# symek/facedeform

Hardware: AMD Instinct MI355X
Metric: deformed Mverts/sec at 256 ctrl pts, 1/2/4/8 MI355X vs host-CPU ref (higher is better)
Workload: dtype f32

## Files before the change

### facedeform_amd/csrc/fd_capi.hip

```cpp
#include <algorithm>
#include <atomic>
#include <cstdarg>
#include <cstdio>
#include <cstdlib>
#include <cstring>
#include <initializer_list>
#include <new>
#include <vector>

#include "fd_internal.h"

using namespace fd;

struct GraphKey {
    int M, kind, term, nparams;
    double params[4];
    const void *A, *rest, *rec32;
};

struct fd_batch;
struct fd_ctx {
    int device = 0;
    hipStream_t own_stream = nullptr;
    hipStream_t stream_ = nullptr;
    int eval_precision = FD_EVAL_FP32;
    int eval_variant = 0;
    int output = FD_OUTPUT_POSITION;
    int solver = FD_SOLVER_AUTO;
    int imported_layers = 0;
    uint64_t rig_build_id = 0;
    const float *rest_src = nullptr;
    bool prefer_lu = false;
    unsigned long long model_gen = 0;
    bool last_spd = false;
    bool last_small = false;
    bool last_nopivot = false;
    bool last_reg = false;

    int M = 0, kind = FD_KERNEL_GAUSSIAN_QNN, term = FD_TERM_LINEAR, nparams = 0;
    double params[4] = {1.0, 5.0, 0.0, 0.0};
    bool points_set = false;
    bool build_pending = false;
    bool built = false;
    bool have_report = false;
    fd_report report{};
    bool have_factor = false;
    bool factor_grouped = false;
    bool deltas_only = false;
    hipGraphExec_t resolve_exec = nullptr;

    int cap_M = 0;
// ... 8 lines not shown
    MfmaTile *d_tiles = nullptr;
    MfmaTileH *d_tiles16 = nullptr;
    double *d_ns = nullptr;
    DevModel *d_model = nullptr;
    DevModel *h_model = nullptr;
    BatchSlot *d_slot = nullptr;
    BatchSlot h_slot{};
    uint64_t alloc_gen = 0;
    hipEvent_t wait_event = nullptr;
    hipStream_t wait_stream = nullptr;
    struct fd_batch *wait_batch = nullptr;
    hipEvent_t tev0 = nullptr, tev_mid = nullptr, tev1 = nullptr;
    ModelHeader *h_header = nullptr;
    int *h_status = nullptr;
    int *d_status_alias = nullptr;
    hipEvent_t status_ev = nullptr;
    hipEvent_t status_poll = nullptr;
    bool status_inflight = false;
    int sticky_rc = FD_OK;

    int64_t cap_N = 0;
    float *d_P = nullptr, *d_dist2 = nullptr, *d_fall = nullptr;
    float *d_tu = nullptr, *d_tv = nullptr, *d_nrm = nullptr;
    int64_t cap_vec = 0, cap_vecP = 0;
    float *d_vec = nullptr, *d_vecP = nullptr;
    int64_t cap_iters = 0;
    int *d_iters = nullptr;
    size_t cap_adj = 0;
    double *d_adj = nullptr;
    int64_t mesh_N = 0, mesh_cap = 0;
    bool mesh_has_dist2 = false, mesh_has_frames = false;
    float *m_P = nullptr, *m_dist2 = nullptr, *m_tu = nullptr, *m_tv = nullptr, *m_nrm = nullptr;
    float *m_out = nullptr, *m_fall = nullptr;

    hipEvent_t ev0 = nullptr, ev_mid = nullptr, ev1 = nullptr;

    hipGraphExec_t build_exec = nullptr;
    bool use_graph = true;
    GraphKey graph_key{}, resolve_key{};
    char err[512] = {0};
};

struct ShotScratch {
    void *d = nullptr;
    size_t cap = 0;
    hipEvent_t consumed_ev = nullptr;
    bool consumed = false;
    hipEvent_t eval_ev = nullptr;
    bool eval_pending = false;
};

struct fd_batch {
    int n = 0;
    int device = 0;
    fd_ctx *ctxs[kMaxBatch] = {};
    uint64_t gens[kMaxBatch] = {};
    BatchSlot *d_slots = nullptr;
    PointSrc src{};
    bool have_src = false;
    hipEvent_t ev0 = nullptr, ev_mid = nullptr, ev1 = nullptr;
    hipGraphExec_t exec = nullptr;
    bool use_graph = true;
    GraphKey key{};
    hipStream_t waited_stream = nullptr;
    hipEvent_t status_ev = nullptr;
    struct SharedSet {
// ... 304 lines not shown
    }
    if (strncmp(prop.gcnArchName, "gfx950", 6) != 0) {
        set_err(nullptr, "fd_create: device %d is %s; kernels are built for gfx950 (MI355X) only",
                dev, prop.gcnArchName);
        delete ctx;
        return nullptr;
    }
    bool ok = true;
    ok = ok && hipEventCreate(&ctx->ev0) == hipSuccess && hipEventCreate(&ctx->ev_mid) == hipSuccess &&
         hipEventCreate(&ctx->ev1) == hipSuccess;
    ok = ok && hipMalloc((void **)&ctx->d_model, sizeof(DevModel)) == hipSuccess;
    ok = ok && hipMalloc((void **)&ctx->d_slot, sizeof(BatchSlot)) == hipSuccess;
    ok = ok && hipHostMalloc((void **)&ctx->h_model, sizeof(DevModel), hipHostMallocDefault) == hipSuccess;
    ok = ok && hipHostMalloc((void **)&ctx->h_header, sizeof(ModelHeader), hipHostMallocDefault) == hipSuccess;
    ok = ok && hipHostMalloc((void **)&ctx->h_status, sizeof(int), hipHostMallocDefault) == hipSuccess;
    if (ok && hipHostGetDevicePointer((void **)&ctx->d_status_alias, ctx->h_status, 0) != hipSuccess) { (void)hipGetLastError(); ctx->d_status_alias = nullptr; }
    ok = ok && hipEventCreateWithFlags(&ctx->status_ev, hipEventDisableTiming) == hipSuccess;
    if (ok) ok = hipMemset(ctx->d_model, 0, sizeof(DevModel)) == hipSuccess;
    if (!ok) {
        set_err(nullptr, "fd_create: device resource allocation failed: %s",
                hipGetErrorString(hipGetLastError()));
        fd_destroy(ctx);
        return nullptr;
    }
    ctx->tev0 = ctx->ev0; ctx->tev_mid = ctx->ev_mid; ctx->tev1 = ctx->ev1;
    return ctx;
}

void fd_destroy(fd_ctx *ctx)
{
    if (!ctx) return;
    (void)hipSetDevice(ctx->device);
    if (ctx->stream_ || ctx->own_stream) (void)hipStreamSynchronize(cur_stream(ctx));
    void *bufs[] = {ctx->d_rest, ctx->d_delta, ctx->d_centres, ctx->d_radii, ctx->d_W, ctx->d_A,
                    ctx->d_X, ctx->d_ipiv, ctx->d_moves, ctx->d_rec32, ctx->d_rec64, ctx->d_tiles, ctx->d_tiles16, ctx->d_ns, ctx->d_model, ctx->d_slot,
                    ctx->d_P, ctx->d_dist2, ctx->d_fall, ctx->d_tu, ctx->d_tv, ctx->d_nrm, ctx->d_vec, ctx->d_vecP, ctx->d_iters, ctx->d_adj,
                    ctx->m_P, ctx->m_dist2, ctx->m_tu, ctx->m_tv, ctx->m_nrm, ctx->m_out, ctx->m_fall};
    for (void *p : bufs) if (p) (void)hipFree(p);
    if (ctx->h_model) (void)hipHostFree(ctx->h_model);
    if (ctx->h_header) (void)hipHostFree(ctx->h_header);
    if (ctx->h_status) (void)hipHostFree(ctx->h_status);
    if (ctx->status_ev) (void)hipEventDestroy(ctx->status_ev);
    if (ctx->build_exec) (void)hipGraphExecDestroy(ctx->build_exec);
    if (ctx->resolve_exec) (void)hipGraphExecDestroy(ctx->resolve_exec);
    if (ctx->ev0) (void)hipEventDestroy(ctx->ev0);
    if (ctx->ev_mid) (void)hipEventDestroy(ctx->ev_mid);
    if (ctx->ev1) (void)hipEventDestroy(ctx->ev1);
    if (ctx->own_stream) (void)hipStreamDestroy(ctx->own_stream);
    delete ctx;
}

int fd_set_stream(fd_ctx *ctx, void *hip_stream)
{
    if (!ctx) return FD_E_INVALID;
    int rc = use_device(ctx);
    if (rc) return rc;
    if (ctx->stream_ || ctx->own_stream) FD_HIP(ctx, hipStreamSynchronize(cur_stream(ctx)));
    ctx->stream_ = (hipStream_t)hip_stream;
    return FD_OK;
}

int fd_synchronize(fd_ctx *ctx)
{
    if (!ctx) return FD_E_INVALID;
    int rc = use_device(ctx);
    if (rc) return rc;
// ... 834 lines not shown
    unsigned char *d_mask = nullptr;
    hipError_t e = hipMalloc((void **)&d_P, sizeof(float) * 3 * (size_t)N);
    if (e == hipSuccess) e = hipMalloc((void **)&d_off, sizeof(int64_t) * (size_t)(N + 1));
    if (e == hipSuccess) e = hipMalloc((void **)&d_nb, sizeof(int) * (size_t)(E > 0 ? E : 1));
    if (e == hipSuccess) e = hipMalloc((void **)&d_mask, (size_t)N);
    if (e == hipSuccess && M > 0) e = hipMalloc((void **)&d_rig, sizeof(float) * 3 * (size_t)M);
    if (e == hipSuccess) e = hipMemcpyAsync(d_P, P, sizeof(float) * 3 * (size_t)N, hipMemcpyHostToDevice, s);
    if (e == hipSuccess) e = hipMemcpyAsync(d_off, offsets, sizeof(int64_t) * (size_t)(N + 1), hipMemcpyHostToDevice, s);
    if (e == hipSuccess && E > 0) e = hipMemcpyAsync(d_nb, neighbours, sizeof(int) * (size_t)E, hipMemcpyHostToDevice, s);
    if (e == hipSuccess && M > 0) e = hipMemcpyAsync(d_rig, rig_xyz, sizeof(float) * 3 * (size_t)M, hipMemcpyHostToDevice, s);
    if (e == hipSuccess) e = launch_capture_islands(d_P, N, d_off, d_nb, d_rig, M, max_edges, d_mask, s);
    if (e == hipSuccess) e = hipMemcpyAsync(mask, d_mask, (size_t)N, hipMemcpyDeviceToHost, s);
    if (e == hipSuccess) e = hipStreamSynchronize(s);
    for (void *p : {(void *)d_P, (void *)d_off, (void *)d_nb, (void *)d_mask, (void *)d_rig}) if (p) (void)hipFree(p);
    if (e != hipSuccess) { set_err(ctx, "fd_capture_islands failed: %s", hipGetErrorString(e)); return FD_E_DEVICE; }
    return FD_OK;
}

void *fd_host_alloc(size_t bytes)
{
    void *p = nullptr;
    if (hipHostMalloc(&p, bytes ? bytes : 1, hipHostMallocDefault) != hipSuccess) {
        set_err(nullptr, "fd_host_alloc(%zu) failed: %s", bytes, hipGetErrorString(hipGetLastError()));
        return nullptr;
    }
    return p;
}

void fd_host_free(void *p)
{
    if (p) (void)hipHostFree(p);
}

int fd_mesh_set(fd_ctx *ctx, int64_t N, const float *P, const float *dist2, const float *tu, const float *tv,
                const float *nrm)
{
    if (!ctx) return FD_E_INVALID;
    if (N <= 0 || !P) { set_err(ctx, "fd_mesh_set: need N > 0 and P"); return FD_E_INVALID; }
    if (!frames_ok(tu, tv, nrm)) { set_err(ctx, "fd_mesh_set: tu, tv, nrm must be all set or all NULL"); return FD_E_INVALID; }
    int rc = use_device(ctx);
    if (rc) return rc;
    ctx->mesh_N = 0;
    if (N > ctx->mesh_cap) {
        if ((rc = dev_alloc(ctx, &ctx->m_P, (size_t)N * 3))) return rc;
        if (ctx->m_dist2) { (void)hipFree(ctx->m_dist2); ctx->m_dist2 = nullptr; }
        if (ctx->m_tu) { (void)hipFree(ctx->m_tu); ctx->m_tu = nullptr; }
        if (ctx->m_tv) { (void)hipFree(ctx->m_tv); ctx->m_tv = nullptr; }
        if (ctx->m_nrm) { (void)hipFree(ctx->m_nrm); ctx->m_nrm = nullptr; }
        if (ctx->m_out) { (void)hipFree(ctx->m_out); ctx->m_out = nullptr; }
        if (ctx->m_fall) { (void)hipFree(ctx->m_fall); ctx->m_fall = nullptr; }
        ctx->mesh_cap = N;
    }
    if (dist2 && !ctx->m_dist2 && (rc = dev_alloc(ctx, &ctx->m_dist2, (size_t)ctx->mesh_cap))) return rc;
    if (tu && !ctx->m_tu) {
        if ((rc = dev_alloc(ctx, &ctx->m_tu, (size_t)ctx->mesh_cap * 3))) return rc;
        if ((rc = dev_alloc(ctx, &ctx->m_tv, (size_t)ctx->mesh_cap * 3))) return rc;
        if ((rc = dev_alloc(ctx, &ctx->m_nrm, (size_t)ctx->mesh_cap * 3))) return rc;
    }
    hipStream_t s = cur_stream(ctx);
    const size_t b3 = sizeof(float) * 3 * (size_t)N, b1 = sizeof(float) * (size_t)N;
    FD_HIP(ctx, hipMemcpyAsync(ctx->m_P, P, b3, hipMemcpyHostToDevice, s));
    if (dist2) FD_HIP(ctx, hipMemcpyAsync(ctx->m_dist2, dist2, b1, hipMemcpyHostToDevice, s));
    if (tu) {
        FD_HIP(ctx, hipMemcpyAsync(ctx->m_tu, tu, b3, hipMemcpyHostToDevice, s));
        FD_HIP(ctx, hipMemcpyAsync(ctx->m_tv, tv, b3, hipMemcpyHostToDevice, s));
        FD_HIP(ctx, hipMemcpyAsync(ctx->m_nrm, nrm, b3, hipMemcpyHostToDevice, s));
    }
    FD_HIP(ctx, hipStreamSynchronize(s));
    ctx->mesh_N = N;
    ctx->mesh_has_dist2 = dist2 != nullptr;
    ctx->mesh_has_frames = tu != nullptr;
    return FD_OK;
}

int64_t fd_mesh_size(const fd_ctx *ctx) { return ctx ? ctx->mesh_N : 0; }

int fd_deform_mesh(fd_ctx *ctx, float *P_out, float *falloff_out, float radius2, float falloffrate)
{
    if (!ctx) return FD_E_INVALID;
    if (ctx->mesh_N <= 0) { set_err(ctx, "fd_deform_mesh: fd_mesh_set has not been called"); return FD_E_INVALID; }
    if (!P_out) { set_err(ctx, "fd_deform_mesh: P_out is NULL"); return FD_E_INVALID; }
    if (!ctx->built && !ctx->build_pending) { set_err(ctx, "fd_deform_mesh: no successfully built model"); return FD_E_NOT_BUILT; }
    int rc = use_device(ctx);
    if (rc) return rc;
    const int64_t N = ctx->mesh_N;
    hipStream_t s = cur_stream(ctx);
    const float *d2 = ctx->mesh_has_dist2 ? ctx->m_dist2 : nullptr;
    const float *tu = ctx->mesh_has_frames ? ctx->m_tu : nullptr, *tv = ctx->mesh_has_frames ? ctx->m_tv : nullptr,
                *nr = ctx->mesh_has_frames ? ctx->m_nrm : nullptr;
    if (host_is_pinned(P_out) && (!falloff_out || host_is_pinned(falloff_out))) {
        void *zo = nullptr, *zf = nullptr;
        bool ok = hipHostGetDevicePointer(&zo, P_out, 0) == hipSuccess;
        if (ok && falloff_out) ok = hipHostGetDevicePointer(&zf, falloff_out, 0) == hipSuccess;
        if (ok) {
            rc = fd_deform_dev_stream(ctx, s, N, ctx->m_P, (float *)zo, d2, (float *)zf, tu, tv, nr, radius2, falloffrate);
            if (rc) return rc;
            FD_HIP(ctx, hipStreamSynchronize(s));
            return FD_OK;
        }
        (void)hipGetLastError();
    }
    if (!ctx->m_out && (rc = dev_alloc(ctx, &ctx->m_out, (size_t)ctx->mesh_cap * 3))) return rc;
    if (falloff_out && !ctx->m_fall && (rc = dev_alloc(ctx, &ctx->m_fall, (size_t)ctx->mesh_cap))) return rc;
    const size_t b3 = sizeof(float) * 3 * (size_t)N, b1 = sizeof(float) * (size_t)N;
    if (falloff_out && (d2 || radius2 < 0.f)) FD_HIP(ctx, hipMemcpyAsync(ctx->m_fall, falloff_out, b1, hipMemcpyHostToDevice, s));
    rc = fd_deform_dev_stream(ctx, s, N, ctx->m_P, ctx->m_out, d2, falloff_out ? ctx->m_fall : nullptr, tu, tv, nr, radius2,
                              falloffrate);
    if (rc) return rc;
    FD_HIP(ctx, hipMemcpyAsync(P_out, ctx->m_out, b3, hipMemcpyDeviceToHost, s));
    if (falloff_out) FD_HIP(ctx, hipMemcpyAsync(falloff_out, ctx->m_fall, b1, hipMemcpyDeviceToHost, s));
    FD_HIP(ctx, hipStreamSynchronize(s));
    return FD_OK;
}

int fd_mesh_capture(fd_ctx *ctx, const int64_t *offsets, const int *neighbours, int M, const float *rig_xyz,
                    int max_edges, int T, const float *tri_xyz, float radius2, int dofalloff, float *dist2_out)
{
    if (!ctx) return FD_E_INVALID;
    const int64_t N = ctx->mesh_N;
    if (N <= 0) { set_err(ctx, "fd_mesh_capture: fd_mesh_set has not been called"); return FD_E_INVALID; }
    if (!offsets || M < 0 || T < 0 || max_edges < 0 || (M > 0 && !rig_xyz) || (T > 0 && !tri_xyz)) {
        set_err(ctx, "fd_mesh_capture: bad sizes or NULL arrays");
        return FD_E_INVALID;
    }
    const int64_t E = offsets[N];
    if (offsets[0] != 0 || E < 0 || (E > 0 && !neighbours)) { set_err(ctx, "fd_mesh_capture: bad adjacency"); return FD_E_INVALID; }
    int rc = use_device(ctx);
    if (rc) return rc;
    if (!ctx->m_dist2 && (rc = dev_alloc(ctx, &ctx->m_dist2, (size_t)ctx->mesh_cap))) return rc;
    hipStream_t s = cur_stream(ctx);
    float *d_rig = nullptr, *d_tri = nullptr;
    int64_t *d_off = nullptr;
    int *d_nb = nullptr;
    unsigned char *d_mask = nullptr;
    hipError_t e = hipMalloc((void **)&d_off, sizeof(int64_t) * (size_t)(N + 1));
    if (e == hipSuccess) e = hipMalloc((void **)&d_nb, sizeof(int) * (size_t)(E > 0 ? E : 1));
    if (e == hipSuccess) e = hipMalloc((void **)&d_mask, (size_t)N);
    if (e == hipSuccess) e = hipMalloc((void **)&d_rig, sizeof(float) * 3 * (size_t)(M > 0 ? M : 1));
    if (e == hipSuccess) e = hipMalloc((void **)&d_tri, sizeof(float) * 9 * (size_t)(T > 0 ? T : 1));
    if (e == hipSuccess) e = hipMemcpyAsync(d_off, offsets, sizeof(int64_t) * (size_t)(N + 1), hipMemcpyHostToDevice, s);
    if (e == hipSuccess && E > 0) e = hipMemcpyAsync(d_nb, neighbours, sizeof(int) * (size_t)E, hipMemcpyHostToDevice, s);
    if (e == hipSuccess && M > 0) e = hipMemcpyAsync(d_rig, rig_xyz, sizeof(float) * 3 * (size_t)M, hipMemcpyHostToDevice, s);
    if (e == hipSuccess && T > 0) e = hipMemcpyAsync(d_tri, tri_xyz, sizeof(float) * 9 * (size_t)T, hipMemcpyHostToDevice, s);
    if (e == hipSuccess) e = launch_capture_islands(ctx->m_P, N, d_off, d_nb, d_rig, M, max_edges, d_mask, s);
    if (e == hipSuccess) e = launch_capture_dist2(ctx->m_P, N, d_mask, d_tri, T, radius2, dofalloff, ctx->m_dist2, s);
    if (e == hipSuccess && dist2_out) e = hipMemcpyAsync(dist2_out, ctx->m_dist2, sizeof(float) * (size_t)N, hipMemcpyDeviceToHost, s);
    if (e == hipSuccess) e = hipStreamSynchronize(s);
    for (void *p : {(void *)d_off, (void *)d_nb, (void *)d_mask, (void *)d_rig, (void *)d_tri}) if (p) (void)hipFree(p);
    if (e != hipSuccess) { (void)hipGetLastError(); set_err(ctx, "fd_mesh_capture failed: %s", hipGetErrorString(e)); return FD_E_DEVICE; }
    ctx->mesh_has_dist2 = true;
    return FD_OK;
}

int fd_mesh_get_dist2(fd_ctx *ctx, float *dist2_out)
{
    if (!ctx || !dist2_out) return FD_E_INVALID;
    if (ctx->mesh_N <= 0 || !ctx->mesh_has_dist2 || !ctx->m_dist2) { set_err(ctx, "fd_mesh_get_dist2: the mesh has no dist2 array"); return FD_E_INVALID; }
    int rc = use_device(ctx);
    if (rc) return rc;
    hipStream_t s = cur_stream(ctx);
    FD_HIP(ctx, hipMemcpyAsync(dist2_out, ctx->m_dist2, sizeof(float) * (size_t)ctx->mesh_N, hipMemcpyDeviceToHost, s));
    FD_HIP(ctx, hipStreamSynchronize(s));
    return FD_OK;
}

static int require_built(fd_ctx *ctx, const char *who)
{
    if (ctx->build_pending) {
        int rc = fd_build_result(ctx, nullptr);
        if (rc) return rc;
    }
    if (!ctx->built) { set_err(ctx, "%s: no successfully built model", who); return FD_E_NOT_BUILT; }
    return FD_OK;
}

int fd_model_centres(const fd_ctx *ctx) { return ctx ? model_centres(ctx) : 0; }

int fd_get_weights(fd_ctx *ctx, double *W, double *radii)
{
    if (!ctx || !W) return FD_E_INVALID;
    int rc = use_device(ctx);
    if (rc) return rc;
    if ((rc = require_built(ctx, "fd_get_weights"))) return rc;
    const int n = model_centres(ctx);
    FD_HIP(ctx, hipMemcpyAsync(W, ctx->d_W, sizeof(double) * 3 * (size_t)(n + 4), hipMemcpyDeviceToHost, cur_stream(ctx)));
    if (radii) FD_HIP(ctx, hipMemcpyAsync(radii, ctx->d_radii, sizeof(double) * (size_t)n, hipMemcpyDeviceToHost, cur_stream(ctx)));
    FD_HIP(ctx, hipStreamSynchronize(cur_stream(ctx)));
    return FD_OK;
}

static size_t model_bytes_for(int M)
{
    return sizeof(ModelHeader) + sizeof(double) * ((size_t)M * 3 + (size_t)M + (size_t)(M + 4) * 3);
}

// ... 1209 lines not shown
}

int fd_batch_set_shared_factor(fd_batch *b, int on)
{
    if (!b) return FD_E_INVALID;
    b->shared_factor = on ? 1 : 0;
    return FD_OK;
}

int fd_batch_last_build_shared_factor(const fd_batch *b) { return b ? b->last_shared_factor : 0; }

const char *fd_shared_ml_build_kernel_name(int M, int layers, int frames) { return ml_shared_kernel_name(M, layers, frames); }

int fd_batch_set_shared_lu(fd_batch *b, int on)
{
    if (!b) return FD_E_INVALID;
    b->shared_lu = on ? 1 : 0;
    return FD_OK;
}

const char *fd_shared_qnn_build_kernel_name(int M, int frames) { return qnn_shared_kernel_name(M, frames); }

int fd_batch_size(const fd_batch *b) { return b ? b->n : 0; }

const char *fd_shared_kernel_name(int M, int frames, int kind)
{
    const bool takes = (kind == FD_KERNEL_THIN_PLATE || kind == FD_KERNEL_GAUSSIAN || kind == FD_KERNEL_GAUSSIAN_QNN) && M > 0 && round_up(M, kRecPad) >= 32 &&
                       frames >= 1 && frames <= kMaxBatch;
    return takes ? shared_kernel_name(round_up(M, kRecPad), frames, kind) : "";
}

}

#include "fd_shot_dev.h"

struct fd_shot_dev {
    fd_ctx *engine = nullptr;
    hipStream_t work = nullptr, copy = nullptr;
    float *d_rig = nullptr;
    size_t cap_rig = 0;
    int M = 0, F = 0;
    float *d_vecs = nullptr;
    int64_t cap_vecs = 0;
    const float *v_in[3] = {nullptr, nullptr, nullptr};
    struct Set {
        float *d = nullptr;
        size_t bytes = 0;
        hipEvent_t eval_ev = nullptr, delivered_ev = nullptr;
        bool delivering = false;
    } sets[2];
    int set_frames = 0;
    int64_t set_Np = 0;
    bool set_fall = false;
    int set_nvec = 0;
    char err[512] = {0};
};

static void shot_err(fd_shot_dev *sd, const char *fmt, ...)
{
    va_list ap;
    va_start(ap, fmt);
    vsnprintf(sd->err, sizeof(sd->err), fmt, ap);
    va_end(ap);
}

#define FD_SHIP(sd, call)                                                                          \
    do {                                                                                           \
        hipError_t e_ = (call);                                                                    \
// ... 135 lines not shown
        }
        (void)hipGetLastError();
        for (auto &st : sd->sets) { if (st.d) (void)hipFree(st.d); st.d = nullptr; }
    }
    shot_err(sd, "hipMalloc of the shot's staging sets failed: %s", hipGetErrorString(hipErrorOutOfMemory));
    return 0;
}

int fd_shot_dev_wait(fd_shot_dev *sd, int set)
{
    if (!sd || set < 0 || set > 1) return FD_E_INVALID;
    if (!sd->sets[set].delivering) return FD_OK;
    sd->sets[set].delivering = false;
    FD_SHIP(sd, hipEventSynchronize(sd->sets[set].delivered_ev));
    return FD_OK;
}

struct ShotMesh { int64_t N; const float *P, *d2, *tu, *tv, *nr; };
static ShotMesh shot_mesh(const fd_ctx *e)
{
    ShotMesh m{e->mesh_N, e->m_P, e->mesh_has_dist2 ? e->m_dist2 : nullptr, nullptr, nullptr, nullptr};
    if (e->mesh_has_frames) { m.tu = e->m_tu; m.tv = e->m_tv; m.nr = e->m_nrm; }
    return m;
}

int fd_shot_dev_eval(fd_shot_dev *sd, fd_batch *b, int set, int fp64, int multilayer, float radius2, float falloffrate)
{
    if (!sd || !b || set < 0 || set > 1) return FD_E_INVALID;
    const int n = b->n;
    if (!sd->sets[set].d || n > sd->set_frames) { shot_err(sd, "fd_shot_dev_eval: no staging set for %d frames", n); return FD_E_INVALID; }
    int rc = fd_shot_dev_wait(sd, set);
    if (rc) return rc;
    const ShotMesh m = shot_mesh(sd->engine);
    if (m.N <= 0 || shot_pad(m.N) != sd->set_Np) { shot_err(sd, "fd_shot_dev_eval: the staging sets were laid out for another mesh"); return FD_E_INVALID; }
    float *P_out[kMaxBatch], *fall[kMaxBatch], *vo[3][kMaxBatch];
    for (int i = 0; i < n; ++i) {
        P_out[i] = shot_slice_P(sd, set, i);
        fall[i] = shot_slice_fall(sd, set, i);
    }
    fd_batch_vectors vec{};
    vec.struct_size = (int)sizeof(vec);
    int which = 0;
    for (int k = 0; k < 3; ++k) {
        if (!sd->v_in[k]) continue;
        for (int i = 0; i < n; ++i) vo[k][i] = shot_slice_vec(sd, set, which, i);
        ++which;
    }
    if (sd->v_in[0]) { vec.N = sd->v_in[0]; vec.N_out = vo[0]; }
    if (sd->v_in[1]) { vec.tu = sd->v_in[1]; vec.tu_out = vo[1]; }
    if (sd->v_in[2]) { vec.tv = sd->v_in[2]; vec.tv_out = vo[2]; }
    const bool with_vec = which > 0;
    if (sd->set_fall && (m.d2 || radius2 < 0.f))
        FD_SHIP(sd, hipMemsetAsync(shot_slice_fall(sd, set, 0), 0, sizeof(float) * (size_t)n * (size_t)sd->set_Np, sd->work));
    float *const *fo = sd->set_fall ? fall : nullptr;
    if (with_vec) {
        auto call = fp64 ? (multilayer ? fd_batch_deform_vectors_shared_ml_fp64_dev : fd_batch_deform_vectors_shared_fp64_dev)
                         : (multilayer ? fd_batch_deform_vectors_shared_ml_dev : fd_batch_deform_vectors_shared_dev);
        rc = call(b, sd->work, m.N, m.P, P_out, m.d2, fo, m.tu, m.tv, m.nr, radius2, falloffrate, &vec);
    } else {
        auto call = fp64 ? (multilayer ? fd_batch_deform_shared_ml_fp64_dev : fd_batch_deform_shared_fp64_dev)
                         : (multilayer ? fd_batch_deform_shared_ml_dev : fd_batch_deform_shared_dev);
        rc = call(b, sd->work, m.N, m.P, P_out, m.d2, fo, m.tu, m.tv, m.nr, radius2, falloffrate);
    }
    if (rc) { shot_err(sd, "%s", b->err); return rc; }
    FD_SHIP(sd, hipEventRecord(sd->sets[set].eval_ev, sd->work));
    return FD_OK;
}

int fd_shot_dev_eval_fp64_over(fd_shot_dev *sd, fd_ctx *ctx, int set, int slot, float radius2, float falloffrate)
{
    if (!sd || !ctx || set < 0 || set > 1 || slot < 0 || slot >= sd->set_frames || !sd->sets[set].d) return FD_E_INVALID;
    const ShotMesh m = shot_mesh(sd->engine);
    fd_vectors vec{};
    vec.struct_size = (int)sizeof(vec);
    int which = 0;
    float *vo[3] = {nullptr, nullptr, nullptr};
    for (int k = 0; k < 3; ++k)
        if (sd->v_in[k]) vo[k] = shot_slice_vec(sd, set, which++, slot);
    if (sd->v_in[0]) { vec.N = sd->v_in[0]; vec.N_out = vo[0]; }
    if (sd->v_in[1]) { vec.tu = sd->v_in[1]; vec.tu_out = vo[1]; }
    if (sd->v_in[2]) { vec.tv = sd->v_in[2]; vec.tv_out = vo[2]; }
    const int before = ctx->eval_precision;
    ctx->eval_precision = FD_EVAL_FP64;
    const int rc = deform_dev_common(ctx, sd->work, m.N, m.P, shot_slice_P(sd, set, slot), m.d2, shot_slice_fall(sd, set, slot), m.tu, m.tv,
                                     m.nr, radius2, falloffrate, which > 0 ? &vec : nullptr);
    ctx->eval_precision = before;
    if (rc) { shot_err(sd, "%s", ctx->err); return rc; }
    FD_SHIP(sd, hipEventRecord(sd->sets[set].eval_ev, sd->work));
    return FD_OK;
}

int fd_shot_dev_deliver(fd_shot_dev *sd, int set, int n, const unsigned char *skip, float *const *P_out, float *const *falloff,
                        float *const *N_out, float *const *tu_out, float *const *tv_out)
{
    if (!sd || set < 0 || set > 1 || n <= 0 || n > sd->set_frames || !P_out || !sd->sets[set].d) return FD_E_INVALID;
    const int64_t N = sd->engine->mesh_N;
    const size_t b3 = sizeof(float) * 3 * (size_t)N, b1 = sizeof(float) * (size_t)N;
    FD_SHIP(sd, hipStreamWaitEvent(sd->copy, sd->sets[set].eval_ev, 0));
    float *const *vt[3] = {N_out, tu_out, tv_out};
    for (int i = 0; i < n; ++i) {
        if (skip && skip[i]) continue;
        if (P_out[i]) FD_SHIP(sd, hipMemcpyAsync(P_out[i], shot_slice_P(sd, set, i), b3, hipMemcpyDeviceToHost, sd->copy));
        if (falloff && falloff[i] && sd->set_fall)
            FD_SHIP(sd, hipMemcpyAsync(falloff[i], shot_slice_fall(sd, set, i), b1, hipMemcpyDeviceToHost, sd->copy));
        int which = 0;
        for (int k = 0; k < 3; ++k) {
            if (!sd->v_in[k]) continue;
            if (vt[k] && vt[k][i]) FD_SHIP(sd, hipMemcpyAsync(vt[k][i], shot_slice_vec(sd, set, which, i), b3, hipMemcpyDeviceToHost, sd->copy));
            ++which;
        }
    }
    FD_SHIP(sd, hipEventRecord(sd->sets[set].delivered_ev, sd->copy));
    sd->sets[set].delivering = true;
    return FD_OK;
}

int fd_shot_dev_vectors_engine(fd_shot_dev *sd, float radius2, float falloffrate, float *N_out, float *tu_out, float *tv_out)
{
    if (!sd || !sd->sets[0].d || sd->set_frames < 1) return FD_E_INVALID;
    int rc = fd_shot_dev_wait(sd, 0);
    if (rc) return rc;
    fd_ctx *e = sd->engine;
    const ShotMesh m = shot_mesh(e);
    fd_vectors vec{};
    vec.struct_size = (int)sizeof(vec);
    int which = 0;
    float *vo[3] = {nullptr, nullptr, nullptr};
    for (int k = 0; k < 3; ++k)
        if (sd->v_in[k]) vo[k] = shot_slice_vec(sd, 0, which++, 0);
    if (which == 0) { shot_err(sd, "fd_shot_dev_vectors_engine: no vectors were set"); return FD_E_INVALID; }
    if (sd->v_in[0]) { vec.N = sd->v_in[0]; vec.N_out = vo[0]; }
    if (sd->v_in[1]) { vec.tu = sd->v_in[1]; vec.tu_out = vo[1]; }
    if (sd->v_in[2]) { vec.tv = sd->v_in[2]; vec.tv_out = vo[2]; }
    hipStream_t s = cur_stream(e);
    if (sd->set_fall && (m.d2 || radius2 < 0.f)) FD_SHIP(sd, hipMemsetAsync(shot_slice_fall(sd, 0, 0), 0, sizeof(float) * (size_t)sd->set_Np, s));
    rc = deform_dev_common(e, s, m.N, m.P, shot_slice_P(sd, 0, 0), m.d2, shot_slice_fall(sd, 0, 0), m.tu, m.tv, m.nr, radius2, falloffrate, &vec);
    if (rc) { shot_err(sd, "%s", e->err); return rc; }
    float *const host[3] = {N_out, tu_out, tv_out};
    const size_t b3 = sizeof(float) * 3 * (size_t)m.N;
    for (int k = 0; k < 3; ++k)
        if (vo[k] && host[k]) FD_SHIP(sd, hipMemcpyAsync(host[k], vo[k], b3, hipMemcpyDeviceToHost, s));
    FD_SHIP(sd, hipStreamSynchronize(s));
    return FD_OK;
}
```

### facedeform_amd/csrc/fd_shot_dev.h

```cpp
#ifndef FD_SHOT_DEV_H
#define FD_SHOT_DEV_H

#include "../../include/facedeform_hip.h"

struct fd_shot_dev;

fd_shot_dev *fd_shot_dev_create(fd_ctx *engine);
void fd_shot_dev_destroy(fd_shot_dev *sd);
const char *fd_shot_dev_error(const fd_shot_dev *sd);
void *fd_shot_dev_work_stream(fd_shot_dev *sd);

int fd_shot_dev_set_rig(fd_shot_dev *sd, const float *rest, const float *deltas, int M, int F);
const float *fd_shot_dev_rest(const fd_shot_dev *sd);
const float *fd_shot_dev_delta(const fd_shot_dev *sd, int frame);
int fd_shot_dev_set_vectors(fd_shot_dev *sd, const float *N, const float *tu, const float *tv);
int fd_shot_dev_reserve(fd_shot_dev *sd, int frames, int want_falloff);
int fd_shot_dev_eval(fd_shot_dev *sd, fd_batch *batch, int set, int fp64, int multilayer, float radius2, float falloffrate);
int fd_shot_dev_eval_fp64_over(fd_shot_dev *sd, fd_ctx *ctx, int set, int slot, float radius2, float falloffrate);
int fd_shot_dev_deliver(fd_shot_dev *sd, int set, int n, const unsigned char *skip, float *const *P_out, float *const *falloff,
                        float *const *N_out, float *const *tu_out, float *const *tv_out);
int fd_shot_dev_wait(fd_shot_dev *sd, int set);
int fd_shot_dev_vectors_engine(fd_shot_dev *sd, float radius2, float falloffrate, float *N_out, float *tu_out, float *tv_out);

#endif
```

### facedeform_amd/csrc/fd_sop_host.cpp

```cpp
#include <cstdio>
#include <cstdlib>
#include <cstring>
#include <new>
#include <string>
#include <vector>

#include "../../include/facedeform_hip.h"
#include "fd_shot_dev.h"

namespace {

enum ParmType { P_STRING, P_ORD, P_FLOAT, P_INT, P_TOGGLE, P_FLOAT2 };

struct ParmDef {
    const char *token;
    ParmType type;
    double def0, def1;
    const char *label;
};

const ParmDef kParms[] = {
    {"group", P_STRING, 0, 0, "Group"},
    {"model", P_ORD, 0, 0, "Model"},
    {"term", P_ORD, 0, 0, "RBF Term"},
// ... 141 lines not shown
{
    const int i = find_parm(token);
    if (!node || i < 0 || !value) return FD_E_INVALID;
    *value = kParms[i].type == P_ORD ? node->ord(i) : (int)node->fval[i][0];
    return FD_OK;
}

const char *fdsop_messages(const fdsop_node *node) { return node ? node->messages.c_str() : ""; }

fd_ctx *fdsop_engine(fdsop_node *node) { return node ? node->engine : nullptr; }

int fdsop_effective_float(const fdsop_node *node, const char *token, double *value)
{
    if (!node || !token || !value) return FD_E_INVALID;
    if (!strcmp(token, "qcoef")) *value = node->e_qcoef;
    else if (!strcmp(token, "zcoef")) *value = node->e_zcoef;
    else if (!strcmp(token, "radius")) *value = node->e_radius;
    else if (!strcmp(token, "lambda")) *value = node->e_lambda;
    else if (!strcmp(token, "layers")) *value = node->e_layers;
    else if (!strcmp(token, "maxedges")) *value = node->e_maxedges;
    else return FD_E_INVALID;
    return FD_OK;
}

struct CookSetup {
    int model_index, term_index, layers, tangent_disp, morph_space, max_edges, kernel_ext, precision_parm, precision, device, M;
    float qcoef, zcoef, radius, lambda, falloffrate;
    double smoothing;
    bool do_tangent_disp, have_blends, morph_inited_this_cook, use_capture, mesh_ready;
    const float *rest_attr;
    int dofalloff_parm;
};

static bool cook_setup(fdsop_node *node, const fdsop_geo *geo, CookSetup &cs)
{
    if (geo->rest_npoints != geo->deform_npoints) {
        node->add(FDSOP_ERROR, "Rest and deform geometry should match.");
        return false;
    }

    const int model_index = cs.model_index = node->ord(find_parm("model"));
    cs.term_index = node->ord(find_parm("term"));
    const float qcoef = cs.qcoef = (float)sys_max(0.1, node->fval[find_parm("qcoef")][0]);
    const float zcoef = cs.zcoef = (float)sys_max(0.1, node->fval[find_parm("zcoef")][0]);
    const float radius = cs.radius = (float)sys_max(0.01, node->fval[find_parm("radius")][0]);
    const int layers = cs.layers = sys_max(1, (int)node->fval[find_parm("layers")][0]);
    const float lambda = cs.lambda = (float)sys_max(0.01, node->fval[find_parm("lambda")][0]);
    const int tangent_disp = cs.tangent_disp = (int)node->fval[find_parm("tangent")][0];
    const int morph_space = cs.morph_space = (int)node->fval[find_parm("morphspace")][0];
    const int max_edges = cs.max_edges = sys_max(1, (int)node->fval[find_parm("maxedges")][0]);
    cs.falloffrate = (float)node->fval[find_parm("falloffrate")][0];
    node->e_qcoef = qcoef; node->e_zcoef = zcoef; node->e_radius = radius; node->e_lambda = lambda;
    node->e_layers = layers; node->e_maxedges = max_edges;
    cs.kernel_ext = node->ord(find_parm("kernel"));
    cs.smoothing = node->fval[find_parm("smoothing")][0];
    const int precision_parm = cs.precision_parm = node->ord(find_parm("precision"));
    const int precision = cs.precision = precision_parm == 1 ? FD_EVAL_FP64 : FD_EVAL_FP32;
    const int device = cs.device = (int)node->fval[find_parm("device")][0];
    (void)model_index;

    const int M = cs.M = (int)geo->rest_npoints;

    const bool do_tangent_disp = cs.do_tangent_disp = tangent_disp && geo->tangentu && geo->tangentv && geo->N;
    if (tangent_disp && !do_tangent_disp)
        node->add(FDSOP_WARNING, "Append PolyFrameSOP and enable tangent[u/v] and N attribute to allow tangent displacement.");

// ... 28 lines not shown
    } else if (morph_space) {
        node->add(FDSOP_WARNING, "No blendshapes found. Ignoring morphspace deformation.");
    }

    if (!node->engine || node->engine_device != device) {
        node->free_shot();
        if (node->engine) { fd_destroy(node->engine); node->engine = nullptr; }
        node->engine_rig_stale = false;
        fd_config cfg = node->cfg;
        cfg.struct_size = (int)sizeof(fd_config);
        cfg.device = device;
        cfg.eval_precision = precision;
        node->engine = fd_create(&cfg);
        node->engine_precision = precision;
        node->engine_device = device;
        if (!node->engine) {
            std::string t = std::string("Can't create the GPU deformation engine: ") + fd_last_error(nullptr);
            node->add(FDSOP_ERROR, t.c_str());
            return false;
        }
    }
    fd_ctx *ctx = node->engine;

    const int dofalloff_parm = cs.dofalloff_parm = (int)node->fval[find_parm("dofalloff")][0];
    const bool want_d2 = geo->dist2 != nullptr;
    const bool use_capture = cs.use_capture = !want_d2 && geo->edge_offsets && geo->rig_ntris >= 0 && (geo->rig_ntris == 0 || geo->rig_tris);
    cs.mesh_ready = false;
    if (geo->npoints > 0) {
        const bool reuse = geo->mesh_unchanged && fd_mesh_size(ctx) == geo->npoints &&
                           node->mesh_had_dist2 == want_d2 && node->mesh_had_frames == do_tangent_disp &&
                           !(node->captured && !use_capture);
        int mrc = FD_OK;
        if (!reuse) {
            mrc = fd_mesh_set(ctx, geo->npoints, geo->P, geo->dist2, do_tangent_disp ? geo->tangentu : nullptr,
                              do_tangent_disp ? geo->tangentv : nullptr, do_tangent_disp ? geo->N : nullptr);
            node->mesh_had_dist2 = want_d2;
            node->mesh_had_frames = do_tangent_disp;
            node->captured = false;
        }
        if (mrc != FD_OK) {
            std::string t = std::string("GPU deformation failed: ") + fd_last_error(ctx);
            node->add(FDSOP_ERROR, t.c_str());
            return false;
        }
        cs.mesh_ready = true;
        if (!use_capture) node->captured = false;
        if (use_capture && (!node->captured || !geo->rig_rest_unchanged)) {
            mrc = fd_mesh_capture(ctx, geo->edge_offsets, geo->edge_neighbours, M > 0 ? M : 0, geo->rest_P, max_edges,
                                  (int)geo->rig_ntris, geo->rig_tris, radius * radius, dofalloff_parm, nullptr);
            if (mrc != FD_OK) {
                node->add(FDSOP_ERROR, "Can't capture geometry with a rig!");
                return false;
            }
            node->captured = true;
        }
    }
    return true;
}

static int cook_select_model(fd_ctx *ctx, const CookSetup &cs)
{
    const int kernel_ext = cs.kernel_ext, model_index = cs.model_index, term_index = cs.term_index, layers = cs.layers;
    const float radius = cs.radius, lambda = cs.lambda, qcoef = cs.qcoef, zcoef = cs.zcoef;
    const double smoothing = cs.smoothing;
    int rc = FD_OK;
    if (kernel_ext == 1 || kernel_ext == 2 || kernel_ext == 3) {
        const int kind = kernel_ext == 1 ? FD_KERNEL_THIN_PLATE : (kernel_ext == 2 ? FD_KERNEL_BIHARMONIC : FD_KERNEL_CUBIC);
        const double p[1] = {smoothing};
        rc = fd_set_kernel(ctx, kind, p, 1);
    } else if (model_index == 1) {
        const double p[3] = {(double)radius, (double)(layers < 8 ? layers : 8), (double)lambda};
        rc = fd_set_kernel(ctx, FD_KERNEL_GAUSSIAN_ML, p, 3);
    } else {
        const double p[3] = {(double)qcoef, (double)zcoef, smoothing};
        rc = fd_set_kernel(ctx, FD_KERNEL_GAUSSIAN_QNN, p, 3);
    }
    const int term = (term_index == 1) ? FD_TERM_CONST : (term_index == 2 ? FD_TERM_ZERO : FD_TERM_LINEAR);
    if (rc == FD_OK) rc = fd_set_term(ctx, term);
    return rc;
}

int fdsop_cook(fdsop_node *node, const fdsop_geo *geo)
{
    if (!node || !geo) return FDSOP_ERROR;
    node->messages.clear();
    node->severity = FDSOP_OK;
    if (geo->npoints < 0 || (geo->npoints > 0 && (!geo->P || !geo->P_out)) || !geo->rest_P || !geo->deform_P) {
        node->add(FDSOP_ERROR, "Invalid geometry arrays.");
        return node->severity;
    }
    struct PassThrough {
        const fdsop_geo *g; bool armed;
        ~PassThrough() {
            if (armed && g->P_out != g->P && g->npoints > 0)
                memcpy(g->P_out, g->P, sizeof(float) * 3 * (size_t)g->npoints);
        }
    } pass{geo, true};

    CookSetup cs;
    if (!cook_setup(node, geo, cs)) return node->severity;
    const int M = cs.M, precision = cs.precision, precision_parm = cs.precision_parm, morph_space = cs.morph_space,
              dofalloff_parm = cs.dofalloff_parm;
    const float radius = cs.radius, falloffrate = cs.falloffrate;
    const bool have_blends = cs.have_blends, morph_inited_this_cook = cs.morph_inited_this_cook, use_capture = cs.use_capture,
               mesh_ready = cs.mesh_ready;
    const float *rest_attr = cs.rest_attr;
    fd_ctx *ctx = node->engine;
    std::vector<float> delta((size_t)(M > 0 ? M : 0) * 3);
    for (int i = 0; i < M; ++i)
        for (int c = 0; c < 3; ++c) delta[3 * (size_t)i + c] = geo->deform_P[3 * (size_t)i + c] - geo->rest_P[3 * (size_t)i + c];

    int rc = cook_select_model(ctx, cs);
    if (rc == FD_OK) {
        rc = FD_E_NOT_BUILT;
        if (M > 0 && geo->rig_rest_unchanged && !node->engine_rig_stale) rc = fd_set_deltas(ctx, delta.data(), M);
        if (rc != FD_OK) {
            rc = M > 0 ? fd_set_points(ctx, geo->rest_P, delta.data(), M) : FD_E_INVALID;
            if (rc == FD_OK) node->engine_rig_stale = false;
        }
    }
    if (rc != FD_OK) {
        node->add(FDSOP_ERROR, "Can't build RBF model.");
        return node->severity;
    }
    fd_report report;
    memset(&report, 0, sizeof(report));
    rc = fd_build(ctx, &report);
    if (report.terminationtype != 1 || rc != FD_OK) {
        node->add(FDSOP_ERROR, "Can't solve the problem.");
        return node->severity;
    }
    int cook_precision = precision;
    if (!geo->rig_rest_unchanged) node->fp64_warned = false;
    if (precision_parm == 0 && !fd_fp32_holds(&report, 1e-5)) {
        cook_precision = FD_EVAL_FP64;
        if (!node->fp64_warned) {
            char t[240];
            snprintf(t, sizeof(t), "fp32 evaluation would not hold 1e-5 of this rig's displacements (error ~%.2g, smallest delta %.2g): "
                                   "evaluating in fp64.", report.fp32_error, report.delta_min);
            node->add(FDSOP_WARNING, t);
            node->fp64_warned = true;
        }
    }
    fd_set_eval_precision(ctx, cook_precision);
    node->last_cook_fp64 = cook_precision == FD_EVAL_FP64;
    char info[200];
    snprintf(info, sizeof(info), "Termination type: %d, Iterations: %d", report.terminationtype, report.iterationscount);
    node->add(FDSOP_MESSAGE, info);

    if (geo->Cd)
        for (int64_t i = 0; i < geo->npoints * 3; ++i) geo->Cd[i] = 1.f;
    if (!geo->dist2 && !(use_capture && node->captured))
        node->add(FDSOP_WARNING, "Can't find distance capture attribute. Won't apply radius nor falloff.");
    if (geo->fd_falloff && geo->npoints > 0) memset(geo->fd_falloff, 0, sizeof(float) * (size_t)geo->npoints);
    const float radius_sqrt = radius * radius;

    pass.armed = false;
    rc = FD_OK;
    if (mesh_ready) rc = fd_deform_mesh(ctx, geo->P_out, geo->fd_falloff, radius_sqrt, falloffrate);
    if (rc == FD_OK && geo->dist2_out && use_capture && node->captured)
        rc = fd_mesh_get_dist2(ctx, geo->dist2_out);
    if (rc != FD_OK) {
        std::string t = std::string("GPU deformation failed: ") + fd_last_error(ctx);
        node->add(FDSOP_ERROR, t.c_str());
        pass.armed = true;
        return node->severity;
    }

    if (morph_space && have_blends && node->morph && fd_morph_is_initialised(node->morph)) {
        bool weights_done = false;
        const int S = fd_morph_shape_count(node->morph);
        if (!fd_morph_is_computed(node->morph)) {
            const int dofalloff = dofalloff_parm;
            const int doclampweight = (int)node->fval[find_parm("doclampweight")][0];
            const float falloffradius = (float)node->fval[find_parm("falloffradius")][0];
            const float weightrange[2] = {(float)node->fval[find_parm("weightrange")][0],
                                          (float)node->fval[find_parm("weightrange")][1]};
            std::vector<double> w((size_t)(S > 0 ? S : 1));
            const bool same_rest = morph_inited_this_cook && rest_attr == geo->P;
            int mrc = fd_morph_set_rest(node->morph, same_rest ? nullptr : rest_attr, 0);
            if (mrc == FD_OK)
                mrc = fd_morph_apply(node->morph, geo->P_out, doclampweight ? weightrange : nullptr,
                                     dofalloff && falloffradius != 0.f, falloffradius, w.data());
            weights_done = mrc == FD_OK;
            if (weights_done) {
                if (geo->weights) memcpy(geo->weights, w.data(), sizeof(double) * (size_t)S);
                if (geo->weights_count) *geo->weights_count = S;
// ... 162 lines not shown
        const bool bad = !shot->deform_P[k] || !shot->P_out[k] || (shot->fd_falloff && !shot->fd_falloff[k]) ||
                         (shot->N_out && !shot->N_out[k]) || (shot->tangentu_out && !shot->tangentu_out[k]) ||
                         (shot->tangentv_out && !shot->tangentv_out[k]);
        if (bad) {
            node->add(FDSOP_ERROR, "Invalid shot arguments.");
            all_frames_error();
            return node->severity;
        }
    }
    if (geo->npoints < 0 || (geo->npoints > 0 && !geo->P) || !geo->rest_P || (shot->N_out && !geo->N) ||
        (shot->tangentu_out && !geo->tangentu) || (shot->tangentv_out && !geo->tangentv)) {
        node->add(FDSOP_ERROR, "Invalid geometry arrays.");
        all_frames_error();
        return node->severity;
    }

    ShotLog log;
    auto finish = [&] {
        node->messages = log.text;
        node->severity = log.severity;
        return node->severity;
    };
    const bool transport = shot_transport(shot);

    if ((F == 1 && !transport) || geo->npoints == 0) {
        cook_frames_sequential(node, geo, shot, 0, F, true, log);
        return finish();
    }

    struct PassAll {
        const fdsop_geo *g; const fdsop_shot *s; bool armed;
        ~PassAll() { if (armed) for (int k = 0; k < s->nframes; ++k) shot_pass_through(g, s, k); }
    } pass{geo, shot, true};
    CookSetup cs;
    bool ok = cook_setup(node, geo, cs);
    int rc = FD_OK;
    if (ok) {
        rc = cook_select_model(node->engine, cs);
        if (rc == FD_OK && cs.M <= 0) rc = FD_E_INVALID;
        if (rc != FD_OK) { node->add(FDSOP_ERROR, "Can't build RBF model."); ok = false; }
    }
    log.take(node, 0);
    if (!ok) {
        all_frames_error();
        return finish();
    }
    pass.armed = false;
    const int M = cs.M;
    const int64_t npoints = geo->npoints;
    if (!geo->rig_rest_unchanged) { node->fp64_warned = false; node->engine_rig_stale = true; }

    if (!node->shot_dev) node->shot_dev = fd_shot_dev_create(node->engine);
    bool batched = node->shot_dev != nullptr && F > 1;
    if (transport && !shot_prepare_vectors(node, geo, shot)) batched = false;
    int G = 0;
    if (node->shot_dev) {
        G = fd_shot_dev_reserve(node->shot_dev, F < FD_MAX_BATCH ? F : FD_MAX_BATCH, shot->fd_falloff != nullptr);
        if (G <= 0) batched = false;
    }
    if (batched) {
        for (int i = node->shot_nctx; i < G; ++i) {
            fd_config cfg = node->cfg;
            cfg.struct_size = (int)sizeof(fd_config);
            cfg.device = cs.device;
            cfg.eval_precision = FD_EVAL_FP32;
            node->shot_ctx[i] = fd_create(&cfg);
// ... 163 lines not shown
```

Before: 63620.

## Overlap chunked mesh upload with RBF build and per-range deformation

Mesh upload now runs asynchronously on a dedicated non-blocking stream, split into up to four ranges with an event recorded per range. The cook path starts the upload, runs the RBF build asynchronously while filling host buffers, and the zero-copy deform launches each range's kernel as soon as that range's event fires. This is meant to hide host-to-device transfer and build latency behind each other. In exchange it adds cross-stream ordering that must be enforced at every consumer of the mesh, plus extra kernel launches.

```diff
diff --git a/facedeform_amd/csrc/fd_capi.hip b/facedeform_amd/csrc/fd_capi.hip
--- a/facedeform_amd/csrc/fd_capi.hip
+++ b/facedeform_amd/csrc/fd_capi.hip
@@ -9,6 +9,7 @@
 #include <vector>
 
 #include "fd_internal.h"
+#include "fd_shot_dev.h"
 
 using namespace fd;
 
@@ -17,6 +18,20 @@
     double params[4];
     const void *A, *rest, *rec32;
 };
+
+constexpr int kMeshMaxRanges = 4;
+constexpr int64_t kMeshRangeMin = 262144;
+static int mesh_ranges(int64_t N, int64_t *start)
+{
+    int64_t L = (N + kMeshMaxRanges - 1) / kMeshMaxRanges;
+    L = (L + 63) / 64 * 64;
+    if (L < kMeshRangeMin) L = kMeshRangeMin;
+    int n = 0;
+    for (int64_t at = 0; at < N; at += L) start[n++] = at;
+    if (n == 0) start[n++] = 0;
+    start[n] = N;
+    return n;
+}
 
 struct fd_batch;
 struct fd_ctx {
@@ -91,6 +106,11 @@
     bool mesh_has_dist2 = false, mesh_has_frames = false;
     float *m_P = nullptr, *m_dist2 = nullptr, *m_tu = nullptr, *m_tv = nullptr, *m_nrm = nullptr;
     float *m_out = nullptr, *m_fall = nullptr;
+    hipStream_t mesh_stream = nullptr;
+    hipEvent_t mesh_ev[kMeshMaxRanges] = {};
+    int mesh_nranges = 0;
+    int64_t mesh_start[kMeshMaxRanges + 1] = {};
+    bool mesh_pending = false;
 
     hipEvent_t ev0 = nullptr, ev_mid = nullptr, ev1 = nullptr;
 
@@ -461,6 +481,8 @@
     if (!ctx) return;
     (void)hipSetDevice(ctx->device);
     if (ctx->stream_ || ctx->own_stream) (void)hipStreamSynchronize(cur_stream(ctx));
+    if (ctx->mesh_stream) { (void)hipStreamSynchronize(ctx->mesh_stream); (void)hipStreamDestroy(ctx->mesh_stream); }
+    for (hipEvent_t ev : ctx->mesh_ev) if (ev) (void)hipEventDestroy(ev);
     void *bufs[] = {ctx->d_rest, ctx->d_delta, ctx->d_centres, ctx->d_radii, ctx->d_W, ctx->d_A,
                     ctx->d_X, ctx->d_ipiv, ctx->d_moves, ctx->d_rec32, ctx->d_rec64, ctx->d_tiles, ctx->d_tiles16, ctx->d_ns, ctx->d_model, ctx->d_slot,
                     ctx->d_P, ctx->d_dist2, ctx->d_fall, ctx->d_tu, ctx->d_tv, ctx->d_nrm, ctx->d_vec, ctx->d_vecP, ctx->d_iters, ctx->d_adj,
@@ -1361,8 +1383,27 @@
     if (p) (void)hipHostFree(p);
 }
 
-int fd_mesh_set(fd_ctx *ctx, int64_t N, const float *P, const float *dist2, const float *tu, const float *tv,
-                const float *nrm)
+}
+
+static int mesh_order(fd_ctx *ctx, hipStream_t s)
+{
+    if (ctx->mesh_pending) FD_HIP(ctx, hipStreamWaitEvent(s, ctx->mesh_ev[ctx->mesh_nranges - 1], 0));
+    return FD_OK;
+}
+
+int fd_mesh_upload_drain(fd_ctx *ctx)
+{
+    if (!ctx) return FD_E_INVALID;
+    if (!ctx->mesh_pending) return FD_OK;
+    ctx->mesh_pending = false;
+    int rc = use_device(ctx);
+    if (rc) return rc;
+    FD_HIP(ctx, hipEventSynchronize(ctx->mesh_ev[ctx->mesh_nranges - 1]));
+    return FD_OK;
+}
+
+int fd_mesh_upload_begin(fd_ctx *ctx, int64_t N, const float *P, const float *dist2, const float *tu, const float *tv,
+                         const float *nrm)
 {
     if (!ctx) return FD_E_INVALID;
     if (N <= 0 || !P) { set_err(ctx, "fd_mesh_set: need N > 0 and P"); return FD_E_INVALID; }
@@ -1370,6 +1411,7 @@
     int rc = use_device(ctx);
     if (rc) return rc;
     ctx->mesh_N = 0;
+    if ((rc = fd_mesh_upload_drain(ctx))) return rc;
     if (N > ctx->mesh_cap) {
         if ((rc = dev_alloc(ctx, &ctx->m_P, (size_t)N * 3))) return rc;
         if (ctx->m_dist2) { (void)hipFree(ctx->m_dist2); ctx->m_dist2 = nullptr; }
@@ -1386,20 +1428,45 @@
         if ((rc = dev_alloc(ctx, &ctx->m_tv, (size_t)ctx->mesh_cap * 3))) return rc;
         if ((rc = dev_alloc(ctx, &ctx->m_nrm, (size_t)ctx->mesh_cap * 3))) return rc;
     }
-    hipStream_t s = cur_stream(ctx);
-    const size_t b3 = sizeof(float) * 3 * (size_t)N, b1 = sizeof(float) * (size_t)N;
-    FD_HIP(ctx, hipMemcpyAsync(ctx->m_P, P, b3, hipMemcpyHostToDevice, s));
-    if (dist2) FD_HIP(ctx, hipMemcpyAsync(ctx->m_dist2, dist2, b1, hipMemcpyHostToDevice, s));
-    if (tu) {
-        FD_HIP(ctx, hipMemcpyAsync(ctx->m_tu, tu, b3, hipMemcpyHostToDevice, s));
-        FD_HIP(ctx, hipMemcpyAsync(ctx->m_tv, tv, b3, hipMemcpyHostToDevice, s));
-        FD_HIP(ctx, hipMemcpyAsync(ctx->m_nrm, nrm, b3, hipMemcpyHostToDevice, s));
-    }
-    FD_HIP(ctx, hipStreamSynchronize(s));
+    if (!ctx->mesh_stream && hipStreamCreateWithFlags(&ctx->mesh_stream, hipStreamNonBlocking) != hipSuccess) {
+        (void)hipGetLastError();
+        ctx->mesh_stream = nullptr;
+    }
+    hipStream_t s = ctx->mesh_stream ? ctx->mesh_stream : cur_stream(ctx);
+    const int R = ctx->mesh_nranges = mesh_ranges(N, ctx->mesh_start);
+    hipError_t e = hipSuccess;
+    for (int k = 0; k < R && e == hipSuccess; ++k) {
+        const size_t at = (size_t)ctx->mesh_start[k], n = (size_t)(ctx->mesh_start[k + 1] - ctx->mesh_start[k]);
+        const size_t b3 = sizeof(float) * 3 * n, b1 = sizeof(float) * n;
+        if (!ctx->mesh_ev[k]) e = hipEventCreateWithFlags(&ctx->mesh_ev[k], hipEventDisableTiming);
+        if (e == hipSuccess) e = hipMemcpyAsync(ctx->m_P + 3 * at, P + 3 * at, b3, hipMemcpyHostToDevice, s);
+        if (e == hipSuccess && dist2) e = hipMemcpyAsync(ctx->m_dist2 + at, dist2 + at, b1, hipMemcpyHostToDevice, s);
+        if (e == hipSuccess && tu) e = hipMemcpyAsync(ctx->m_tu + 3 * at, tu + 3 * at, b3, hipMemcpyHostToDevice, s);
+        if (e == hipSuccess && tu) e = hipMemcpyAsync(ctx->m_tv + 3 * at, tv + 3 * at, b3, hipMemcpyHostToDevice, s);
+        if (e == hipSuccess && tu) e = hipMemcpyAsync(ctx->m_nrm + 3 * at, nrm + 3 * at, b3, hipMemcpyHostToDevice, s);
+        if (e == hipSuccess) e = hipEventRecord(ctx->mesh_ev[k], s);
+    }
+    if (e != hipSuccess) {
+        (void)hipStreamSynchronize(s);
+        (void)hipGetLastError();
+        set_err(ctx, "fd_mesh_set: the upload failed: %s", hipGetErrorString(e));
+        return FD_E_DEVICE;
+    }
+    ctx->mesh_pending = true;
     ctx->mesh_N = N;
     ctx->mesh_has_dist2 = dist2 != nullptr;
     ctx->mesh_has_frames = tu != nullptr;
     return FD_OK;
+}
+
+extern "C" {
+
+int fd_mesh_set(fd_ctx *ctx, int64_t N, const float *P, const float *dist2, const float *tu, const float *tv,
+                const float *nrm)
+{
+    int rc = fd_mesh_upload_begin(ctx, N, P, dist2, tu, tv, nrm);
+    if (rc == FD_OK && (rc = fd_mesh_upload_drain(ctx))) ctx->mesh_N = 0;
+    return rc;
 }
 
 int64_t fd_mesh_size(const fd_ctx *ctx) { return ctx ? ctx->mesh_N : 0; }
@@ -1422,13 +1489,28 @@
         bool ok = hipHostGetDevicePointer(&zo, P_out, 0) == hipSuccess;
         if (ok && falloff_out) ok = hipHostGetDevicePointer(&zf, falloff_out, 0) == hipSuccess;
         if (ok) {
-            rc = fd_deform_dev_stream(ctx, s, N, ctx->m_P, (float *)zo, d2, (float *)zf, tu, tv, nr, radius2, falloffrate);
-            if (rc) return rc;
+            const bool ranged = ctx->mesh_pending;
+            const int R = ranged ? ctx->mesh_nranges : 1;
+            for (int k = 0; k < R; ++k) {
+                const int64_t at = ranged ? ctx->mesh_start[k] : 0, n = ranged ? ctx->mesh_start[k + 1] - at : N;
+                if (ranged && hipStreamWaitEvent(s, ctx->mesh_ev[k], 0) != hipSuccess) {
+                    set_err(ctx, "fd_deform_mesh: hipStreamWaitEvent failed: %s", hipGetErrorString(hipGetLastError()));
+                    rc = FD_E_DEVICE;
+                    break;
+                }
+                rc = fd_deform_dev_stream(ctx, s, n, ctx->m_P + 3 * at, (float *)zo + 3 * at, d2 ? d2 + at : nullptr,
+                                          zf ? (float *)zf + at : nullptr, tu ? tu + 3 * at : nullptr, tv ? tv + 3 * at : nullptr,
+                                          nr ? nr + 3 * at : nullptr, radius2, falloffrate);
+                if (rc) break;
+            }
+            if (rc) { (void)hipStreamSynchronize(s); return rc; }
             FD_HIP(ctx, hipStreamSynchronize(s));
+            ctx->mesh_pending = false;
             return FD_OK;
         }
         (void)hipGetLastError();
     }
+    if ((rc = mesh_order(ctx, s))) return rc;
     if (!ctx->m_out && (rc = dev_alloc(ctx, &ctx->m_out, (size_t)ctx->mesh_cap * 3))) return rc;
     if (falloff_out && !ctx->m_fall && (rc = dev_alloc(ctx, &ctx->m_fall, (size_t)ctx->mesh_cap))) return rc;
     const size_t b3 = sizeof(float) * 3 * (size_t)N, b1 = sizeof(float) * (size_t)N;
@@ -1439,6 +1521,7 @@
     FD_HIP(ctx, hipMemcpyAsync(P_out, ctx->m_out, b3, hipMemcpyDeviceToHost, s));
     if (falloff_out) FD_HIP(ctx, hipMemcpyAsync(falloff_out, ctx->m_fall, b1, hipMemcpyDeviceToHost, s));
     FD_HIP(ctx, hipStreamSynchronize(s));
+    ctx->mesh_pending = false;
     return FD_OK;
 }
 
@@ -1458,6 +1541,7 @@
     if (rc) return rc;
     if (!ctx->m_dist2 && (rc = dev_alloc(ctx, &ctx->m_dist2, (size_t)ctx->mesh_cap))) return rc;
     hipStream_t s = cur_stream(ctx);
+    if ((rc = mesh_order(ctx, s))) return rc;
     float *d_rig = nullptr, *d_tri = nullptr;
     int64_t *d_off = nullptr;
     int *d_nb = nullptr;
@@ -1477,6 +1561,7 @@
     if (e == hipSuccess) e = hipStreamSynchronize(s);
     for (void *p : {(void *)d_off, (void *)d_nb, (void *)d_mask, (void *)d_rig, (void *)d_tri}) if (p) (void)hipFree(p);
     if (e != hipSuccess) { (void)hipGetLastError(); set_err(ctx, "fd_mesh_capture failed: %s", hipGetErrorString(e)); return FD_E_DEVICE; }
+    ctx->mesh_pending = false;
     ctx->mesh_has_dist2 = true;
     return FD_OK;
 }
@@ -1488,8 +1573,10 @@
     int rc = use_device(ctx);
     if (rc) return rc;
     hipStream_t s = cur_stream(ctx);
+    if ((rc = mesh_order(ctx, s))) return rc;
     FD_HIP(ctx, hipMemcpyAsync(dist2_out, ctx->m_dist2, sizeof(float) * (size_t)ctx->mesh_N, hipMemcpyDeviceToHost, s));
     FD_HIP(ctx, hipStreamSynchronize(s));
+    ctx->mesh_pending = false;
     return FD_OK;
 }
 
@@ -2765,8 +2852,6 @@
 
 }
 
-#include "fd_shot_dev.h"
-
 struct fd_shot_dev {
     fd_ctx *engine = nullptr;
     hipStream_t work = nullptr, copy = nullptr;
@@ -2968,6 +3053,7 @@
     int rc = fd_shot_dev_wait(sd, set);
     if (rc) return rc;
     const ShotMesh m = shot_mesh(sd->engine);
+    if ((rc = mesh_order(sd->engine, sd->work))) { shot_err(sd, "%s", sd->engine->err); return rc; }
     if (m.N <= 0 || shot_pad(m.N) != sd->set_Np) { shot_err(sd, "fd_shot_dev_eval: the staging sets were laid out for another mesh"); return FD_E_INVALID; }
     float *P_out[kMaxBatch], *fall[kMaxBatch], *vo[3][kMaxBatch];
     for (int i = 0; i < n; ++i) {
@@ -3007,6 +3093,7 @@
 {
     if (!sd || !ctx || set < 0 || set > 1 || slot < 0 || slot >= sd->set_frames || !sd->sets[set].d) return FD_E_INVALID;
     const ShotMesh m = shot_mesh(sd->engine);
+    if (mesh_order(sd->engine, sd->work) != FD_OK) { shot_err(sd, "%s", sd->engine->err); return FD_E_DEVICE; }
     fd_vectors vec{};
     vec.struct_size = (int)sizeof(vec);
     int which = 0;
@@ -3069,6 +3156,7 @@
     if (sd->v_in[1]) { vec.tu = sd->v_in[1]; vec.tu_out = vo[1]; }
     if (sd->v_in[2]) { vec.tv = sd->v_in[2]; vec.tv_out = vo[2]; }
     hipStream_t s = cur_stream(e);
+    if ((rc = mesh_order(e, s))) { shot_err(sd, "%s", e->err); return rc; }
     if (sd->set_fall && (m.d2 || radius2 < 0.f)) FD_SHIP(sd, hipMemsetAsync(shot_slice_fall(sd, 0, 0), 0, sizeof(float) * (size_t)sd->set_Np, s));
     rc = deform_dev_common(e, s, m.N, m.P, shot_slice_P(sd, 0, 0), m.d2, shot_slice_fall(sd, 0, 0), m.tu, m.tv, m.nr, radius2, falloffrate, &vec);
     if (rc) { shot_err(sd, "%s", e->err); return rc; }
diff --git a/facedeform_amd/csrc/fd_shot_dev.h b/facedeform_amd/csrc/fd_shot_dev.h
--- a/facedeform_amd/csrc/fd_shot_dev.h
+++ b/facedeform_amd/csrc/fd_shot_dev.h
@@ -22,4 +22,7 @@
 int fd_shot_dev_wait(fd_shot_dev *sd, int set);
 int fd_shot_dev_vectors_engine(fd_shot_dev *sd, float radius2, float falloffrate, float *N_out, float *tu_out, float *tv_out);
 
+int fd_mesh_upload_begin(fd_ctx *ctx, int64_t N, const float *P, const float *dist2, const float *tu, const float *tv, const float *nrm);
+int fd_mesh_upload_drain(fd_ctx *ctx);
+
 #endif
diff --git a/facedeform_amd/csrc/fd_sop_host.cpp b/facedeform_amd/csrc/fd_sop_host.cpp
--- a/facedeform_amd/csrc/fd_sop_host.cpp
+++ b/facedeform_amd/csrc/fd_sop_host.cpp
@@ -197,6 +197,11 @@
     int dofalloff_parm;
 };
 
+struct UploadGuard {
+    fdsop_node *node;
+    ~UploadGuard() { if (node->engine) (void)fd_mesh_upload_drain(node->engine); }
+};
+
 static bool cook_setup(fdsop_node *node, const fdsop_geo *geo, CookSetup &cs)
 {
     if (geo->rest_npoints != geo->deform_npoints) {
@@ -291,8 +296,8 @@
                            !(node->captured && !use_capture);
         int mrc = FD_OK;
         if (!reuse) {
-            mrc = fd_mesh_set(ctx, geo->npoints, geo->P, geo->dist2, do_tangent_disp ? geo->tangentu : nullptr,
-                              do_tangent_disp ? geo->tangentv : nullptr, do_tangent_disp ? geo->N : nullptr);
+            mrc = fd_mesh_upload_begin(ctx, geo->npoints, geo->P, geo->dist2, do_tangent_disp ? geo->tangentu : nullptr,
+                                       do_tangent_disp ? geo->tangentv : nullptr, do_tangent_disp ? geo->N : nullptr);
             node->mesh_had_dist2 = want_d2;
             node->mesh_had_frames = do_tangent_disp;
             node->captured = false;
@@ -356,6 +361,7 @@
         }
     } pass{geo, true};
 
+    UploadGuard upload{node};
     CookSetup cs;
     if (!cook_setup(node, geo, cs)) return node->severity;
     const int M = cs.M, precision = cs.precision, precision_parm = cs.precision_parm, morph_space = cs.morph_space,
@@ -384,7 +390,11 @@
     }
     fd_report report;
     memset(&report, 0, sizeof(report));
-    rc = fd_build(ctx, &report);
+    rc = fd_build_async(ctx);
+    if (geo->Cd)
+        for (int64_t i = 0; i < geo->npoints * 3; ++i) geo->Cd[i] = 1.f;
+    if (geo->fd_falloff && geo->npoints > 0) memset(geo->fd_falloff, 0, sizeof(float) * (size_t)geo->npoints);
+    if (rc == FD_OK) rc = fd_build_result(ctx, &report);
     if (report.terminationtype != 1 || rc != FD_OK) {
         node->add(FDSOP_ERROR, "Can't solve the problem.");
         return node->severity;
@@ -407,11 +417,8 @@
     snprintf(info, sizeof(info), "Termination type: %d, Iterations: %d", report.terminationtype, report.iterationscount);
     node->add(FDSOP_MESSAGE, info);
 
-    if (geo->Cd)
-        for (int64_t i = 0; i < geo->npoints * 3; ++i) geo->Cd[i] = 1.f;
     if (!geo->dist2 && !(use_capture && node->captured))
         node->add(FDSOP_WARNING, "Can't find distance capture attribute. Won't apply radius nor falloff.");
-    if (geo->fd_falloff && geo->npoints > 0) memset(geo->fd_falloff, 0, sizeof(float) * (size_t)geo->npoints);
     const float radius_sqrt = radius * radius;
 
     pass.armed = false;
@@ -640,6 +647,7 @@
         const fdsop_geo *g; const fdsop_shot *s; bool armed;
         ~PassAll() { if (armed) for (int k = 0; k < s->nframes; ++k) shot_pass_through(g, s, k); }
     } pass{geo, shot, true};
+    UploadGuard upload{node};
     CookSetup cs;
     bool ok = cook_setup(node, geo, cs);
     int rc = FD_OK;
```

After: 63920, median of 4. Within noise of the previous version (+0.5%).
